# manikya7022/Continual-Learning-for-Dynamic-Video-Quality-Enhancement

Hardware: AMD Instinct MI355X
Metric: train frames/sec (2x SR, T=3, 540p->1080p) (higher is better)
Workload: dtype bf16

## Files before the change

continual-learning-for-dynamic-video-quality-enhancement_amd/csrc/aggregate.hip:

```cpp
#include "common.h"

namespace nvq {

__device__ __forceinline__ float sigmoidf_(float x) { return 1.f / (1.f + __expf(-x)); }

__device__ __forceinline__ float4 plane_reduce4b(float4 v, float4* buf, int C4, int npl) {
    __syncthreads();
    buf[threadIdx.x] = v;
    __syncthreads();
    float4 s = make_float4(0.f, 0.f, 0.f, 0.f);
    if ((int)threadIdx.x < C4)
        for (int k = 0; k < npl; ++k) {
            const float4 t = buf[k * C4 + threadIdx.x];
            s.x += t.x; s.y += t.y; s.z += t.z; s.w += t.w;
        }
    return s;
}

static inline int tsum_blocks_host(int H, int W) {
    int nb = ceil_div((long)H * W, 1024);
    if (nb > 256) nb = 256;
    if (nb < 1) nb = 1;
    return nb;
}
// ... 30 lines not shown
            const long pu = p0 + u * stride;
            if (pu >= HW) break;
            const long pix = base + pu;
            float mx = -3.4e38f;
#pragma unroll
            for (int t = 0; t < TMAX; ++t) mx = fmaxf(mx, lg[u][t]);
            float den = 0.f;
#pragma unroll
            for (int t = 0; t < TMAX; ++t) {
                lg[u][t] = t < T ? __expf(lg[u][t] - mx) : 0.f;
                den += lg[u][t];
            }
            const float inv = 1.f / den;
            float4 o = make_float4(0.f, 0.f, 0.f, 0.f);
#pragma unroll
            for (int t = 0; t < TMAX; ++t) {
                if (t < T) {
                    const float a = lg[u][t] * inv;
                    o.x += v[u][t].x * a; o.y += v[u][t].y * a; o.z += v[u][t].z * a; o.w += v[u][t].w * a;
                    if (c4 == 0) attn[pix * attn_ld + t] = a;
                }
            }
            if (c4 == 0)
                for (int t = T; t < attn_ld; ++t) attn[pix * attn_ld + t] = 0.f;
            stx4(weighted, pix * weighted_ld + 4 * c4, WB, o);
            gsum.x += o.x; gsum.y += o.y; gsum.z += o.z; gsum.w += o.w;
        }
    }
    const float4 r = plane_reduce4b(gsum, buf, C4, npl);
    if ((int)threadIdx.x < C4)
        st4(gap_partial + ((size_t)blockIdx.y * gridDim.x + blockIdx.x) * C + 4 * c4, r);
}

template <bool ALLB, bool WB>
__global__ __launch_bounds__(256) void tsum_bwd_kernel(const float* __restrict__ dweighted, int dweighted_ld,
                                                       const float* __restrict__ dgap_pix,
                                                       const float* __restrict__ aligned, int aligned_ld,
                                                       const float* __restrict__ attn, int attn_ld, int T, int C,
                                                       long HW, float* __restrict__ daligned, int daligned_ld,
                                                       float* __restrict__ dlogits, int dlogits_ld, long total,
                                                       int aligned_bf16_, int daligned_bf16_) {
    const int aligned_bf16 = ALLB ? 1 : aligned_bf16_, daligned_bf16 = ALLB ? 1 : daligned_bf16_;
    const long gid = blockIdx.x * 256L + threadIdx.x;
    if (gid >= total) return;
    const int C4 = C >> 2;
    const long pix = idiv(gid, C4, total);
    const int c4 = (int)(gid - pix * C4);
    const int n = (int)idiv(pix, HW, total);
    float4 dw = ldx4(dweighted, pix * dweighted_ld + 4 * c4, WB);
    if (dgap_pix) {
        const float4 gp = ld4(dgap_pix + (size_t)n * C + 4 * c4);
        dw.x += gp.x; dw.y += gp.y; dw.z += gp.z; dw.w += gp.w;
    }
    float a[NVQ_MAX_T], dot[NVQ_MAX_T];
    float sdot = 0.f;
#pragma unroll
    for (int t = 0; t < NVQ_MAX_T; ++t) {
        a[t] = 0.f; dot[t] = 0.f;
        if (t < T) {
            a[t] = attn[pix * attn_ld + t];
            const float4 v = ldx4(aligned, (size_t)pix * aligned_ld + t * C + 4 * c4, aligned_bf16);
            stx4(daligned, (size_t)pix * daligned_ld + t * C + 4 * c4, daligned_bf16,
                 make_float4(dw.x * a[t], dw.y * a[t], dw.z * a[t], dw.w * a[t]));
            dot[t] = group_sum(dw.x * v.x + dw.y * v.y + dw.z * v.z + dw.w * v.w, C4);
            sdot += a[t] * dot[t];
        }
    }
    if (c4 == 0) {
#pragma unroll
        for (int t = 0; t < NVQ_MAX_T; ++t)
            if (t < T) dlogits[pix * dlogits_ld + t] = a[t] * (dot[t] - sdot);
        for (int t = T; t < dlogits_ld; ++t) dlogits[pix * dlogits_ld + t] = 0.f;
    }
}

__global__ __launch_bounds__(256) void cbam_channel_kernel(const float* __restrict__ gap_partial, int nblk, int C,
                                                           int R, long HW, const float* __restrict__ w1,
                                                           const float* __restrict__ w2, float* __restrict__ gap,
                                                           float* __restrict__ hid, float* __restrict__ ca) {
    __shared__ float sg[256];
    __shared__ float sh[64];
    const int n = blockIdx.x, c = threadIdx.x;
    if (c < C) {
        double s = 0.0;
        const float* p = gap_partial + (size_t)n * nblk * C + c;
        for (int b = 0; b < nblk; ++b) s += (double)p[(size_t)b * C];
        const float g = (float)(s / (double)HW);
        sg[c] = g;
        gap[(size_t)n * C + c] = g;
    }
    __syncthreads();
    if (c < R) {
        float s = 0.f;
        for (int k = 0; k < C; ++k) s += w1[c * C + k] * sg[k];
        s = fmaxf(s, 0.f);
        sh[c] = s;
        hid[(size_t)n * R + c] = s;
    }
    __syncthreads();
    if (c < C) {
        float s = 0.f;
        for (int r = 0; r < R; ++r) s += w2[c * R + r] * sh[r];
        ca[(size_t)n * C + c] = sigmoidf_(s);
    }
}

template <bool XB>
__global__ __launch_bounds__(256) void cbam_pool_kernel(const float* __restrict__ x, int x_ld,
                                                        const float* __restrict__ ca, int C, long HW,
                                                        float* __restrict__ sm, int* __restrict__ amax, long total) {
    const long gid = blockIdx.x * 256L + threadIdx.x;
    if (gid >= total) return;
    const int C4 = C >> 2;
    const long pix = idiv(gid, C4, total);
    const int c4 = (int)(gid - pix * C4);
    const int n = (int)idiv(pix, HW, total);
    const float4 v = ldx4(x, pix * x_ld + 4 * c4, XB);
    const float4 a = ld4(ca + (size_t)n * C + 4 * c4);
    const float e[4] = {v.x * a.x, v.y * a.y, v.z * a.z, v.w * a.w};
    const float s = group_sum(e[0] + e[1] + e[2] + e[3], C4);
    float best = e[0];
    int bi = 4 * c4;
#pragma unroll
    for (int k = 1; k < 4; ++k)
        if (e[k] > best) { best = e[k]; bi = 4 * c4 + k; }
    for (int o = C4 >> 1; o > 0; o >>= 1) {
        const float ob = __shfl_xor(best, o, 64);
        const int oi = __shfl_xor(bi, o, 64);
        if (ob > best || (ob == best && oi < bi)) { best = ob; bi = oi; }
    }
    if (c4 == 0) {
        sm[pix * 2] = s / (float)C;
        sm[pix * 2 + 1] = best;
        amax[pix] = bi;
    }
}

constexpr int SP_T = 16;
constexpr int SP_H = SP_T + 6;

__global__ __launch_bounds__(256) void cbam_sa_kernel(const float* __restrict__ sm, const float* __restrict__ w7,
                                                      int H, int W, int tilesX, float* __restrict__ sa) {
    __shared__ float tile[2][SP_H][SP_H + 1];
    __shared__ float wl[98];
    const int n = blockIdx.y;
    const int ty0 = (blockIdx.x / tilesX) * SP_T, tx0 = (blockIdx.x % tilesX) * SP_T;
    if (threadIdx.x < 98) wl[threadIdx.x] = w7[threadIdx.x];
    for (int i = threadIdx.x; i < SP_H * SP_H; i += 256) {
        const int hy = i / SP_H, hx = i % SP_H;
        const int gy = ty0 + hy - 3, gx = tx0 + hx - 3;
        float a = 0.f, b = 0.f;
        if (gy >= 0 && gy < H && gx >= 0 && gx < W) {
            const size_t pix = (size_t)(n * H + gy) * W + gx;
            a = sm[pix * 2];
            b = sm[pix * 2 + 1];
        }
        tile[0][hy][hx] = a;
        tile[1][hy][hx] = b;
    }
    __syncthreads();
    const int py = threadIdx.x / SP_T, px = threadIdx.x % SP_T;
    const int gy = ty0 + py, gx = tx0 + px;
    if (gy >= H || gx >= W) return;
    float s = 0.f;
#pragma unroll
    for (int ch = 0; ch < 2; ++ch)
#pragma unroll
        for (int ky = 0; ky < 7; ++ky)
#pragma unroll
            for (int kx = 0; kx < 7; ++kx) s += wl[(ch * 7 + ky) * 7 + kx] * tile[ch][py + ky][px + kx];
    sa[(size_t)(n * H + gy) * W + gx] = sigmoidf_(s);
}

template <bool XB>
__global__ __launch_bounds__(256) void cbam_apply_kernel(const float* __restrict__ x, int x_ld,
                                                         const float* __restrict__ ca, const float* __restrict__ sa,
                                                         int C, long HW, float* __restrict__ out, int out_ld,
                                                         int out_coff, int out_bf16, long total) {
    const long gid = blockIdx.x * 256L + threadIdx.x;
    if (gid >= total) return;
    const int C4 = C >> 2;
    const long pix = idiv(gid, C4, total);
    const int c4 = (int)(gid - pix * C4);
    const int n = (int)idiv(pix, HW, total);
    const float4 v = ldx4(x, pix * x_ld + 4 * c4, XB);
    const float4 a = ld4(ca + (size_t)n * C + 4 * c4);
    const float s = sa[pix];
    const float4 o = make_float4(v.x * a.x * s, v.y * a.y * s, v.z * a.z * s, v.w * a.w * s);
    if (out_bf16) {
        typedef __bf16 bf16x4_t __attribute__((ext_vector_type(4)));
        *reinterpret_cast<bf16x4_t*>(reinterpret_cast<__bf16*>(out) + pix * out_ld + out_coff + 4 * c4) =
            (bf16x4_t){(__bf16)o.x, (__bf16)o.y, (__bf16)o.z, (__bf16)o.w};
    } else {
        st4(out + pix * out_ld + out_coff + 4 * c4, o);
    }
}

template <bool XB>
__global__ __launch_bounds__(256) void cbam_bwd_pre_kernel(const float* __restrict__ dout, int dout_ld, int dout_coff,
                                                           const float* __restrict__ x, int x_ld,
                                                           const float* __restrict__ ca, const float* __restrict__ sa,
                                                           int C, long HW, float* __restrict__ dpre, long total) {
    const long gid = blockIdx.x * 256L + threadIdx.x;
    if (gid >= total) return;
    const int C4 = C >> 2;
    const long pix = idiv(gid, C4, total);
    const int c4 = (int)(gid - pix * C4);
    const int n = (int)idiv(pix, HW, total);
    const float4 g = ldx4(dout, pix * dout_ld + dout_coff + 4 * c4, XB);
    const float4 v = ldx4(x, pix * x_ld + 4 * c4, XB);
    const float4 a = ld4(ca + (size_t)n * C + 4 * c4);
    const float d = group_sum(g.x * v.x * a.x + g.y * v.y * a.y + g.z * v.z * a.z + g.w * v.w * a.w, C4);
    if (c4 == 0) {
        const float s = sa[pix];
        dpre[pix] = d * s * (1.f - s);
    }
}

template <bool WG>
__global__ __launch_bounds__(256) void cbam_bwd_conv_kernel(const float* __restrict__ dpre,
                                                            const float* __restrict__ sm,
                                                            const float* __restrict__ w7, int H, int W, int tilesX,
                                                            float* __restrict__ dsm, float* __restrict__ part) {
    __shared__ float dtile[SP_H][SP_H + 1];
    __shared__ float stile[2][SP_H][SP_H + 1];
    __shared__ float wl[98];
    const int n = blockIdx.y;
    const int ty0 = (blockIdx.x / tilesX) * SP_T, tx0 = (blockIdx.x % tilesX) * SP_T;
    if (threadIdx.x < 98) wl[threadIdx.x] = w7[threadIdx.x];
    for (int i = threadIdx.x; i < SP_H * SP_H; i += 256) {
        const int hy = i / SP_H, hx = i % SP_H;
        const int gy = ty0 + hy - 3, gx = tx0 + hx - 3;
        float d = 0.f, a = 0.f, b = 0.f;
        if (gy >= 0 && gy < H && gx >= 0 && gx < W) {
            const size_t pix = (size_t)(n * H + gy) * W + gx;
            d = dpre[pix];
            if constexpr (WG) {
                a = sm[pix * 2];
                b = sm[pix * 2 + 1];
            }
        }
        dtile[hy][hx] = d;
        if constexpr (WG) {
            stile[0][hy][hx] = a;
            stile[1][hy][hx] = b;
        }
    }
    __syncthreads();
    const int py = threadIdx.x / SP_T, px = threadIdx.x % SP_T;
    const int gy = ty0 + py, gx = tx0 + px;
    if (gy < H && gx < W) {
        float s0 = 0.f, s1 = 0.f;
#pragma unroll
        for (int ky = 0; ky < 7; ++ky)
#pragma unroll
            for (int kx = 0; kx < 7; ++kx) {
                const float d = dtile[py + 6 - ky][px + 6 - kx];
                s0 += wl[ky * 7 + kx] * d;
                s1 += wl[49 + ky * 7 + kx] * d;
            }
        const size_t pix = (size_t)(n * H + gy) * W + gx;
        dsm[pix * 2] = s0;
        dsm[pix * 2 + 1] = s1;
    }
    if (WG && threadIdx.x < 98) {
        const int ch = threadIdx.x / 49, ky = (threadIdx.x % 49) / 7, kx = threadIdx.x % 7;
        float s = 0.f;
        for (int yy = 0; yy < SP_T; ++yy)
            for (int xx = 0; xx < SP_T; ++xx) s += stile[ch][yy + ky][xx + kx] * dtile[yy + 3][xx + 3];
        part[((size_t)blockIdx.y * gridDim.x + blockIdx.x) * 98 + threadIdx.x] = s;
    }
}

template <bool XB>
__global__ __launch_bounds__(256) void cbam_bwd_scale_kernel(const float* __restrict__ dout, int dout_ld, int dout_coff,
                                                             const float* __restrict__ x, int x_ld,
                                                             const float* __restrict__ ca, const float* __restrict__ sa,
                                                             const float* __restrict__ dsm, const int* __restrict__ amax,
                                                             int C, long HW, float* __restrict__ dx, int dx_ld,
                                                             float* __restrict__ dca_partial) {
    __shared__ float4 buf[256];
    const int C4 = C >> 2;
    const int npl = 256 / C4;
    const int c4 = threadIdx.x % C4, pl = threadIdx.x / C4;
    const int n = blockIdx.y;
    const long base = (long)n * HW;
    const float4 a = ld4(ca + (size_t)n * C + 4 * c4);
    const float invC = 1.f / (float)C;
    float4 acc = make_float4(0.f, 0.f, 0.f, 0.f);
    for (long p = (long)blockIdx.x * npl + pl; p < HW; p += (long)gridDim.x * npl) {
        const long pix = base + p;
        const float4 g = ldx4(dout, pix * dout_ld + dout_coff + 4 * c4, XB);
        const float4 v = ldx4(x, pix * x_ld + 4 * c4, XB);
        const float s = sa[pix];
        const float d0 = dsm[pix * 2] * invC, d1 = dsm[pix * 2 + 1];
        const int am = amax[pix] - 4 * c4;
        float4 dxc;
        dxc.x = g.x * s + d0 + (am == 0 ? d1 : 0.f);
        dxc.y = g.y * s + d0 + (am == 1 ? d1 : 0.f);
        dxc.z = g.z * s + d0 + (am == 2 ? d1 : 0.f);
        dxc.w = g.w * s + d0 + (am == 3 ? d1 : 0.f);
        stx4(dx, pix * dx_ld + 4 * c4, XB, make_float4(dxc.x * a.x, dxc.y * a.y, dxc.z * a.z, dxc.w * a.w));
        acc.x += dxc.x * v.x; acc.y += dxc.y * v.y; acc.z += dxc.z * v.z; acc.w += dxc.w * v.w;
    }
    const float4 r = plane_reduce4b(acc, buf, C4, npl);
    if ((int)threadIdx.x < C4)
        st4(dca_partial + ((size_t)n * gridDim.x + blockIdx.x) * C + 4 * c4, r);
}

template <bool WG>
__global__ __launch_bounds__(256) void cbam_bwd_channel_kernel(const float* __restrict__ dca_partial, int nblk, int C,
                                                               int R, int N, long HW, const float* __restrict__ w1,
                                                               const float* __restrict__ w2, const float* __restrict__ gap,
                                                               const float* __restrict__ hid, const float* __restrict__ ca,
                                                               float* __restrict__ dw1, float* __restrict__ dw2,
                                                               float* __restrict__ dgap_pix, int accumulate) {
    __shared__ float dz2[256];
    __shared__ float dz1[16];
    __shared__ float sh[16];
    const int c = threadIdx.x;
    float a1[16], a2[16];
#pragma unroll
    for (int r = 0; r < 16; ++r) { a1[r] = 0.f; a2[r] = 0.f; }
    __shared__ double sp[256];
    const int parts = 256 / C;
    for (int n = 0; n < N; ++n) {
        __syncthreads();
        {
            const int cc = c % C, part = c / C;
            double s = 0.0;
            if (part < parts) {
                const float* p = dca_partial + (size_t)n * nblk * C + cc;
                for (int b = part; b < nblk; b += parts) s += (double)p[(size_t)b * C];
            }
            sp[c] = s;
        }
        __syncthreads();
        float z = 0.f;
        if (c < C) {
            double s = 0.0;
            for (int k = 0; k < parts; ++k) s += sp[k * C + c];
            const float cav = ca[(size_t)n * C + c];
            z = (float)s * cav * (1.f - cav);
        }
        dz2[c] = z;
        if (c < R) sh[c] = hid[(size_t)n * R + c];
        __syncthreads();
        if (c < R) {
            float s = 0.f;
            for (int k = 0; k < C; ++k) s += w2[k * R + c] * dz2[k];
            dz1[c] = sh[c] > 0.f ? s : 0.f;
        }
        __syncthreads();
        if (c < C) {
            const float gv = gap[(size_t)n * C + c];
            float dg = 0.f;
#pragma unroll
            for (int r = 0; r < 16; ++r)
                if (r < R) {
                    if constexpr (WG) {
                        a2[r] += z * sh[r];
                        a1[r] += dz1[r] * gv;
                    }
                    dg += w1[r * C + c] * dz1[r];
                }
            dgap_pix[(size_t)n * C + c] = dg / (float)HW;
        }
    }
    if (WG && c < C) {
#pragma unroll
        for (int r = 0; r < 16; ++r)
            if (r < R) {
                dw2[c * R + r] = accumulate ? dw2[c * R + r] + a2[r] : a2[r];
                dw1[r * C + c] = accumulate ? dw1[r * C + c] + a1[r] : a1[r];
            }
    }
}

static bool pow2_c4(int C) {
    const int c4 = C >> 2;
    return C % 4 == 0 && c4 >= 1 && c4 <= 64 && (c4 & (c4 - 1)) == 0;
}

}

using namespace nvq;

extern "C" {

int nvq_tsum_blocks(int H, int W) { return tsum_blocks_host(H, W); }

int nvq_tsum_forward(const float* aligned, int aligned_ld, const float* logits, int logits_ld, int T, int C,
                     int N, int H, int W, float* attn, int attn_ld, float* weighted, int weighted_ld,
                     float* gap_partial, int aligned_bf16, int weighted_bf16, void* stream) {
    NVQ_REQUIRE(pow2_c4(C), "tsum_forward: C %d must be a power of two in [4,256]", C);
    NVQ_REQUIRE(T >= 1 && T <= NVQ_MAX_T && logits_ld >= T && attn_ld >= T, "tsum_forward: T %d", T);
    NVQ_REQUIRE(aligned_ld % 4 == 0 && weighted_ld % 4 == 0 && aligned_ld >= T * C, "tsum_forward: ld");
    const dim3 grid(tsum_blocks_host(H, W), N);
    with_bools([&](auto SMALL, auto AB, auto WB) {
        constexpr int M = SMALL() ? 4 : NVQ_MAX_T, U = SMALL() ? 4 : 2;
        hipLaunchKernelGGL((tsum_fwd_kernel<M, U, AB(), WB()>), grid, dim3(256), 0, (hipStream_t)stream, aligned, aligned_ld, logits,
                           logits_ld, T, C, (long)H * W, attn, attn_ld, weighted, weighted_ld, gap_partial);
    }, T <= 4, aligned_bf16, weighted_bf16);
    return check_launch("tsum_forward");
}

int nvq_tsum_backward(const float* dweighted, int dweighted_ld, const float* dgap_pix, const float* aligned,
                      int aligned_ld, const float* attn, int attn_ld, int T, int C, int N, int H, int W,
                      float* daligned, int daligned_ld, float* dlogits, int dlogits_ld, int aligned_bf16,
                      int daligned_bf16, int dweighted_bf16, void* stream) {
    NVQ_REQUIRE(pow2_c4(C), "tsum_backward: C %d must be a power of two in [4,256]", C);
    NVQ_REQUIRE(T >= 1 && T <= NVQ_MAX_T && dlogits_ld >= T && attn_ld >= T, "tsum_backward: T %d", T);
    NVQ_REQUIRE(aligned_ld % 4 == 0 && dweighted_ld % 4 == 0 && daligned_ld % 4 == 0, "tsum_backward: ld");
    const long total = (long)N * H * W * (C / 4);
    with_bools([&](auto AB, auto WB) {
        hipLaunchKernelGGL((tsum_bwd_kernel<AB(), WB()>), dim3(ceil_div(total, 256)), dim3(256), 0, (hipStream_t)stream, dweighted,
                           dweighted_ld, dgap_pix, aligned, aligned_ld, attn, attn_ld, T, C, (long)H * W, daligned, daligned_ld, dlogits,
                           dlogits_ld, total, aligned_bf16, daligned_bf16);
    }, aligned_bf16 && daligned_bf16, dweighted_bf16);
    return check_launch("tsum_backward");
}

int nvq_cbam_channel(const float* gap_partial, int nblk, int C, int R, int N, int HW, const float* w1,
                     const float* w2, float* gap, float* hid, float* ca, void* stream) {
    NVQ_REQUIRE(C <= 256 && R >= 1 && R <= 16, "cbam_channel: C %d R %d", C, R);
    hipLaunchKernelGGL(cbam_channel_kernel, dim3(N), dim3(256), 0, (hipStream_t)stream, gap_partial, nblk, C, R,
                       (long)HW, w1, w2, gap, hid, ca);
    return check_launch("cbam_channel");
}

int nvq_cbam_pool(const float* x, int x_ld, const float* ca, int C, int N, int H, int W, float* sm, int* amax,
                  int x_bf16, void* stream) {
    NVQ_REQUIRE(pow2_c4(C) && x_ld % 4 == 0, "cbam_pool: C %d must be a power of two in [4,256]", C);
    const long total = (long)N * H * W * (C / 4);
    if (x_bf16)
        hipLaunchKernelGGL(cbam_pool_kernel<true>, dim3(ceil_div(total, 256)), dim3(256), 0, (hipStream_t)stream, x, x_ld, ca, C,
                           (long)H * W, sm, amax, total);
    else
        hipLaunchKernelGGL(cbam_pool_kernel<false>, dim3(ceil_div(total, 256)), dim3(256), 0, (hipStream_t)stream, x, x_ld, ca, C,
                           (long)H * W, sm, amax, total);
    return check_launch("cbam_pool");
}

int nvq_cbam_spatial_apply(const float* x, int x_ld, const float* ca, const float* sm, const float* w7, int C,
                           int N, int H, int W, float* sa, float* out, int out_ld, int out_coff, int out_bf16,
                           int x_bf16, void* stream) {
    NVQ_REQUIRE(C % 4 == 0 && x_ld % 4 == 0 && out_ld % 4 == 0 && out_coff % 4 == 0, "cbam_spatial_apply: alignment");
    const int tilesX = (W + SP_T - 1) / SP_T, tilesY = (H + SP_T - 1) / SP_T;
    hipStream_t s = (hipStream_t)stream;
    hipLaunchKernelGGL(cbam_sa_kernel, dim3(tilesX * tilesY, N), dim3(256), 0, s, sm, w7, H, W, tilesX, sa);
    int rc = check_launch("cbam_sa");
    if (rc) return rc;
    const long total = (long)N * H * W * (C / 4);
    if (x_bf16)
        hipLaunchKernelGGL(cbam_apply_kernel<true>, dim3(ceil_div(total, 256)), dim3(256), 0, s, x, x_ld, ca, sa, C, (long)H * W,
                           out, out_ld, out_coff, out_bf16, total);
    else
        hipLaunchKernelGGL(cbam_apply_kernel<false>, dim3(ceil_div(total, 256)), dim3(256), 0, s, x, x_ld, ca, sa, C, (long)H * W,
                           out, out_ld, out_coff, out_bf16, total);
    return check_launch("cbam_apply");
}

int nvq_cbam_bwd_spatial_pre(const float* dout, int dout_ld, int dout_coff, const float* x, int x_ld,
                             const float* ca, const float* sa, int C, int N, int H, int W, float* dpre,
                             int x_bf16, void* stream) {
    NVQ_REQUIRE(pow2_c4(C) && x_ld % 4 == 0 && dout_ld % 4 == 0 && dout_coff % 4 == 0,
                "cbam_bwd_spatial_pre: C %d must be a power of two in [4,256]", C);
    const long total = (long)N * H * W * (C / 4);
    if (x_bf16)
        hipLaunchKernelGGL(cbam_bwd_pre_kernel<true>, dim3(ceil_div(total, 256)), dim3(256), 0, (hipStream_t)stream, dout, dout_ld,
                           dout_coff, x, x_ld, ca, sa, C, (long)H * W, dpre, total);
    else
        hipLaunchKernelGGL(cbam_bwd_pre_kernel<false>, dim3(ceil_div(total, 256)), dim3(256), 0, (hipStream_t)stream, dout, dout_ld,
                           dout_coff, x, x_ld, ca, sa, C, (long)H * W, dpre, total);
    return check_launch("cbam_bwd_spatial_pre");
}

int nvq_cbam_bwd_spatial_conv_ex(const float* dpre, const float* sm, const float* w7, int N, int H, int W, float* dsm,
                                 float* dw7, float* workspace, size_t workspace_bytes, int accumulate, int flags, void* stream) {
    NVQ_REQUIRE((flags & ~NVQ_NO_WGRAD) == 0, "cbam_bwd_spatial_conv_ex: flags %d", flags);
    const bool wg = !(flags & NVQ_NO_WGRAD);
    const int tilesX = (W + SP_T - 1) / SP_T, tilesY = (H + SP_T - 1) / SP_T;
    const int nblk = tilesX * tilesY * N;
    hipStream_t s = (hipStream_t)stream;
    if (!wg) {
        hipLaunchKernelGGL(cbam_bwd_conv_kernel<false>, dim3(tilesX * tilesY, N), dim3(256), 0, s, dpre, sm, w7, H, W, tilesX,
                           dsm, workspace);
        return check_launch("cbam_bwd_spatial_conv");
    }
    if ((size_t)nblk * 98 * sizeof(float) > workspace_bytes) { set_error("cbam_bwd_spatial_conv: workspace"); return NVQ_EWORKSPACE; }
    hipLaunchKernelGGL(cbam_bwd_conv_kernel<true>, dim3(tilesX * tilesY, N), dim3(256), 0, s, dpre, sm, w7, H, W, tilesX, dsm,
                       workspace);
    int rc = check_launch("cbam_bwd_spatial_conv");
    if (rc) return rc;
    return launch_reduce_partials(workspace, nblk, 98, 1.f, dw7, accumulate, s);
}

int nvq_cbam_bwd_spatial_conv(const float* dpre, const float* sm, const float* w7, int N, int H, int W, float* dsm,
                              float* dw7, float* workspace, size_t workspace_bytes, int accumulate, void* stream) {
    return nvq_cbam_bwd_spatial_conv_ex(dpre, sm, w7, N, H, W, dsm, dw7, workspace, workspace_bytes, accumulate, 0, stream);
}

int nvq_cbam_bwd_scale(const float* dout, int dout_ld, int dout_coff, const float* x, int x_ld, const float* ca,
                       const float* sa, const float* dsm, const int* amax, int C, int N, int H, int W, float* dx,
                       int dx_ld, float* dca_partial, int x_bf16, void* stream) {
    NVQ_REQUIRE(pow2_c4(C) && x_ld % 4 == 0 && dout_ld % 4 == 0 && dout_coff % 4 == 0 && dx_ld % 4 == 0,
                "cbam_bwd_scale: C %d must be a power of two in [4,256]", C);
    if (x_bf16)
        hipLaunchKernelGGL(cbam_bwd_scale_kernel<true>, dim3(tsum_blocks_host(H, W), N), dim3(256), 0, (hipStream_t)stream, dout,
                           dout_ld, dout_coff, x, x_ld, ca, sa, dsm, amax, C, (long)H * W, dx, dx_ld, dca_partial);
    else
        hipLaunchKernelGGL(cbam_bwd_scale_kernel<false>, dim3(tsum_blocks_host(H, W), N), dim3(256), 0, (hipStream_t)stream, dout,
                           dout_ld, dout_coff, x, x_ld, ca, sa, dsm, amax, C, (long)H * W, dx, dx_ld, dca_partial);
    return check_launch("cbam_bwd_scale");
}

int nvq_cbam_bwd_channel_ex(const float* dca_partial, int nblk, int C, int R, int N, int HW, const float* w1,
                            const float* w2, const float* gap, const float* hid, const float* ca, float* dw1,
                            float* dw2, float* dgap_pix, int accumulate, int flags, void* stream) {
    NVQ_REQUIRE((flags & ~NVQ_NO_WGRAD) == 0, "cbam_bwd_channel_ex: flags %d", flags);
    NVQ_REQUIRE(C <= 256 && R >= 1 && R <= 16, "cbam_bwd_channel: C %d R %d", C, R);
    if (flags & NVQ_NO_WGRAD)
        hipLaunchKernelGGL(cbam_bwd_channel_kernel<false>, dim3(1), dim3(256), 0, (hipStream_t)stream, dca_partial, nblk, C, R, N,
                           (long)HW, w1, w2, gap, hid, ca, dw1, dw2, dgap_pix, accumulate);
    else
        hipLaunchKernelGGL(cbam_bwd_channel_kernel<true>, dim3(1), dim3(256), 0, (hipStream_t)stream, dca_partial, nblk, C, R, N,
                           (long)HW, w1, w2, gap, hid, ca, dw1, dw2, dgap_pix, accumulate);
    return check_launch("cbam_bwd_channel");
}

int nvq_cbam_bwd_channel(const float* dca_partial, int nblk, int C, int R, int N, int HW, const float* w1,
                         const float* w2, const float* gap, const float* hid, const float* ca, float* dw1,
                         float* dw2, float* dgap_pix, int accumulate, void* stream) {
    return nvq_cbam_bwd_channel_ex(dca_partial, nblk, C, R, N, HW, w1, w2, gap, hid, ca, dw1, dw2, dgap_pix, accumulate, 0, stream);
}

}
```

continual-learning-for-dynamic-video-quality-enhancement_amd/csrc/common.h:

```cpp
#pragma once
#include <hip/hip_runtime.h>
#include <stdarg.h>
#include <stdio.h>
#include <type_traits>
#include "../../include/nvq.h"

namespace nvq {

void set_error(const char* fmt, ...);

inline int check_launch(const char* what) {
    hipError_t e = hipGetLastError();
    if (e != hipSuccess) {
        set_error("%s: %s", what, hipGetErrorString(e));
        return NVQ_ELAUNCH;
    }
    return NVQ_OK;
}

#define NVQ_REQUIRE(cond, ...)            \
    do {                                  \
        if (!(cond)) {                    \
            nvq::set_error(__VA_ARGS__);  \
            return NVQ_EINVAL;            \
// ... 2 lines not shown

inline bool aligned16(const void* p) { return (reinterpret_cast<uintptr_t>(p) & 15) == 0; }
inline bool aligned8(const void* p) { return (reinterpret_cast<uintptr_t>(p) & 7) == 0; }
inline bool aligned4(const void* p) { return (reinterpret_cast<uintptr_t>(p) & 3) == 0; }
inline int ceil_div(long a, long b) { return (int)((a + b - 1) / b); }

template <bool... Bs, class F>
inline void with_bools(F&& f) {
    f(std::bool_constant<Bs>{}...);
}
template <bool... Bs, class F, class... Rest>
inline void with_bools(F&& f, bool b, Rest... rest) {
    if (b) with_bools<Bs..., true>(f, rest...);
    else with_bools<Bs..., false>(f, rest...);
}

template <int... Vs>
struct one_of {
    int v;
    explicit one_of(int v_) : v(v_) {}
};
template <class... Ks, class F, class... Rest>
inline int with_consts(const char*, F&&, bool, Rest...);
template <class... Ks, class F, class... Rest>
inline int with_consts(const char*, F&&, one_of<>, Rest...);
template <class... Ks, class F, int V, int... Vs, class... Rest>
inline int with_consts(const char*, F&&, one_of<V, Vs...>, Rest...);

template <class... Ks, class F>
inline int with_consts(const char*, F&& f) {
    f(Ks{}...);
    return NVQ_OK;
}
template <class... Ks, class F, class... Rest>
inline int with_consts(const char* what, F&& f, bool b, Rest... rest) {
    return b ? with_consts<Ks..., std::true_type>(what, f, rest...) : with_consts<Ks..., std::false_type>(what, f, rest...);
}
template <class... Ks, class F, class... Rest>
inline int with_consts(const char* what, F&&, one_of<> a, Rest...) {
    set_error("%s: no kernel form for the value %d", what, a.v);
    return NVQ_EINVAL;
}
template <class... Ks, class F, int V, int... Vs, class... Rest>
inline int with_consts(const char* what, F&& f, one_of<V, Vs...> a, Rest... rest) {
    return a.v == V ? with_consts<Ks..., std::integral_constant<int, V>>(what, f, rest...)
                    : with_consts<Ks...>(what, f, one_of<Vs...>(a.v), rest...);
}

typedef float f32x4 __attribute__((ext_vector_type(4)));

__device__ __forceinline__ float4 ld4(const float* p) { return *reinterpret_cast<const float4*>(p); }
__device__ __forceinline__ void st4(float* p, float4 v) { *reinterpret_cast<float4*>(p) = v; }

typedef __bf16 bf16x8 __attribute__((ext_vector_type(8)));
typedef __bf16 bf16x4 __attribute__((ext_vector_type(4)));

__device__ __forceinline__ float4 ldx4(const float* base, size_t idx, int is_bf16) {
    if (is_bf16) {
        const bf16x4 v = *reinterpret_cast<const bf16x4*>(reinterpret_cast<const __bf16*>(base) + idx);
        return make_float4((float)v[0], (float)v[1], (float)v[2], (float)v[3]);
    }
    return ld4(base + idx);
}
__device__ __forceinline__ void stx4(float* base, size_t idx, int is_bf16, float4 v) {
    if (is_bf16)
        *reinterpret_cast<bf16x4*>(reinterpret_cast<__bf16*>(base) + idx) =
            (bf16x4){(__bf16)v.x, (__bf16)v.y, (__bf16)v.z, (__bf16)v.w};
    else
        st4(base + idx, v);
}

__device__ __forceinline__ long idiv(long a, int d, long total) {
    return total <= 0xffffffffL ? (long)((unsigned)a / (unsigned)d) : a / d;
}
__device__ __forceinline__ long idiv(long a, long d, long total) {
    return (total <= 0xffffffffL && d <= 0xffffffffL) ? (long)((unsigned)a / (unsigned)d) : a / d;
}

__device__ __forceinline__ float group_sum(float v, int width) {
    for (int o = width >> 1; o > 0; o >>= 1) v += __shfl_xor(v, o, 64);
    return v;
}

__device__ __forceinline__ float block_sum_256(float v, float* scratch) {
    v = group_sum(v, 64);
    const int wave = threadIdx.x >> 6;
    __syncthreads();
    if ((threadIdx.x & 63) == 0) scratch[wave] = v;
    __syncthreads();
    return scratch[0] + scratch[1] + scratch[2] + scratch[3];
}

__device__ __forceinline__ int xcd_tile(int bid, int n) {
    const int q = n >> 3, r = n & 7, x = bid & 7;
    return x * q + (x < r ? x : r) + (bid >> 3);
}

int launch_reduce_partials(const float* part, int nblk, int K, float alpha, float* out,
                           int accumulate, hipStream_t s);

}
```

continual-learning-for-dynamic-video-quality-enhancement_amd/csrc/conv_igemm.hip:

```cpp
#include "conv_common.h"
#include "flat.h"

namespace nvq {

constexpr int KC = 16;
constexpr int XS_LD = 20;

__device__ __forceinline__ float pack_f32_elem(const float* __restrict__ w, int cout_w, int cin_w, int taps, int transpose,
                                               int cout_keep, int NT, int nkc, long idx) {
    long t = idx;
    const int j = t & 3; t >>= 2;
    const int n = t % NT; t /= NT;
    const int g = t & 3; t >>= 2;
    const int tap = t % taps; t /= taps;
    const int kc = t % nkc; t /= nkc;
    const int cz = (int)t;
    const int co = cz * NT + n;
    const int ch = kc * KC + 4 * g + j;
    float v = 0.f;
    if (!transpose) {
        if (co < cout_w && ch < cin_w) v = w[((long)co * cin_w + ch) * taps + tap];
    } else {
        if (co < cout_keep && ch < cout_w) v = w[((long)ch * cin_w + co) * taps + (taps - 1 - tap)];
    }
// ... 339 lines not shown
            }
            for (; k < nsplit; k += WR_Q) s4[0] += (double)part[(size_t)k * total + idx];
        }
        sh[q][e] = (s4[0] + s4[1]) + (s4[2] + s4[3]);
        __syncthreads();
        if (q == 0 && idx < total) {
            double sum = 0.0;
#pragma unroll
            for (int u = 0; u < WR_Q; ++u) sum += sh[u][e];
            long t = idx;
            const int col = t % WG_C; t /= WG_C;
            const int cil = t % WG_C; t /= WG_C;
            const int tap = t % taps; t /= taps;
            const int coc = t % nco;
            const int cic = (int)(t / nco);
            const int ci = cic * WG_C + cil, co = coc * WG_C + col;
            if (ci < cin_w && co < cout) {
                const float v = alpha * (float)sum;
                const long o = ((long)co * cin_w + ci) * taps + tap;
                dw[o] = accumulate ? dw[o] + v : v;
            }
        }
        __syncthreads();
    }
}

__global__ __launch_bounds__(256) void wgrad_reduce_kernel(const float* __restrict__ part, int nsplit, int nci, int nco,
                                                           int taps, int cout, int cin_w, float alpha, int accumulate,
                                                           float* __restrict__ dw, int wblocks, const float* __restrict__ bp,
                                                           float* __restrict__ dbias) {
    __shared__ double sh[WR_Q][WR_E];
    wgrad_reduce_body(part, nsplit, nci, nco, taps, cout, cin_w, alpha, accumulate, dw, wblocks, bp, dbias, (int)blockIdx.x, sh);
}

constexpr int WR_MAX_JOBS = 16;
struct WgradReduceTable { nvq_wgrad_reduce_job j[WR_MAX_JOBS]; };
__global__ __launch_bounds__(256) void wgrad_reduce_batch_kernel(const WgradReduceTable t) {
    __shared__ double sh[WR_Q][WR_E];
    const nvq_wgrad_reduce_job& j = t.j[blockIdx.y];
    const long total = (long)j.nci * j.nco * j.taps * WG_C * WG_C;
    const int bblk = j.dbias ? (j.cout + 3) / 4 : 0;
    long nblk = (total + WR_E - 1) / WR_E;
    if (nblk > (long)gridDim.x - bblk) nblk = (long)gridDim.x - bblk;
    if ((int)blockIdx.x >= nblk + bblk) return;
    wgrad_reduce_body(j.part, j.nsplit, j.nci, j.nco, j.taps, j.cout, j.cin_w, j.alpha, j.accumulate, j.dw, (int)nblk,
                      j.bias_part, j.dbias, (int)blockIdx.x, sh);
}

static int launch_wgrad_reduce_bias(const float* part, int nsplit, int nci, int nco, int taps, int cout, int cin_w, float alpha,
                                    int accumulate, float* dw, const float* bias_part, float* dbias, hipStream_t s) {
    const long total = (long)nci * nco * taps * WG_C * WG_C;
    int nblk = ceil_div(total, WR_E);
    if (nblk > 4096) nblk = 4096;
    const int bblk = dbias ? ceil_div(cout, 4) : 0;
    hipLaunchKernelGGL(wgrad_reduce_kernel, dim3(nblk + bblk), dim3(256), 0, s, part, nsplit, nci, nco, taps, cout, cin_w, alpha,
                       accumulate, dw, nblk, bias_part, dbias);
    return check_launch("conv_wgrad_reduce");
}
int launch_wgrad_reduce(const float* part, int nsplit, int nci, int nco, int taps, int cout, int cin_w, float alpha,
                        int accumulate, float* dw, hipStream_t s) {
    return launch_wgrad_reduce_bias(part, nsplit, nci, nco, taps, cout, cin_w, alpha, accumulate, dw, nullptr, nullptr, s);
}

__global__ __launch_bounds__(256) void colsum_kernel(const float* __restrict__ x, int ld, int coff,
                                                     int C, int CP, long npix,
                                                     float* __restrict__ part) {
    __shared__ float red[256];
    const int c = threadIdx.x % CP;
    const int pl = threadIdx.x / CP;
    const int lanes = 256 / CP;
    float s = 0.f;
    if (c < C)
        for (long p = (long)blockIdx.x * lanes + pl; p < npix; p += (long)gridDim.x * lanes)
            s += x[p * ld + coff + c];
    red[threadIdx.x] = s;
    __syncthreads();
    if (pl == 0 && c < C) {
        float t = 0.f;
        for (int k = 0; k < lanes; ++k) t += red[k * CP + c];
        part[(long)blockIdx.x * C + c] = t;
    }
}

__global__ __launch_bounds__(256) void reduce_partials_kernel(const float* __restrict__ part, int nblk, int K,
                                                              float alpha, float* __restrict__ out, int accumulate) {
    const int k = blockIdx.x * 4 + (threadIdx.x >> 6);
    const int lane = threadIdx.x & 63;
    if (k >= K) return;
    double s = 0.0;
    for (int b = lane; b < nblk; b += 64) s += (double)part[(long)b * K + k];
    s = wave_sum(s);
    if (lane == 0) {
        const float v = alpha * (float)s;
        out[k] = accumulate ? out[k] + v : v;
    }
}

int launch_reduce_partials(const float* part, int nblk, int K, float alpha, float* out,
                           int accumulate, hipStream_t s) {
    hipLaunchKernelGGL(reduce_partials_kernel, dim3(ceil_div(K, 4)), dim3(256), 0, s, part, nblk,
                       K, alpha, out, accumulate);
    return check_launch("reduce_partials");
}

static int colsum_impl(const float* x, int ld, int coff, int C, long npix, float alpha, float* out,
                       float* ws, size_t ws_bytes, int accumulate, hipStream_t s) {
    NVQ_REQUIRE(C >= 1 && C <= 256, "colsum: C=%d out of range", C);
    int CP = 1;
    while (CP < C) CP <<= 1;
    const int lanes = 256 / CP;
    int nblk = ceil_div(npix, (long)lanes * 8);
    if (nblk > 512) nblk = 512;
    if (nblk < 1) nblk = 1;
    if ((size_t)nblk * C * sizeof(float) > ws_bytes) {
        set_error("colsum: workspace too small");
        return NVQ_EWORKSPACE;
    }
    hipLaunchKernelGGL(colsum_kernel, dim3(nblk), dim3(256), 0, s, x, ld, coff, C, CP, npix, ws);
    int rc = check_launch("colsum");
    if (rc) return rc;
    return launch_reduce_partials(ws, nblk, C, alpha, out, accumulate, s);
}

}

using namespace nvq;

extern "C" {

size_t nvq_conv_pack_floats(int cout, int cin_store, int ksize, int math) {
    if (math == NVQ_MATH_BF16) return pack_floats_bf16(cout, cin_store, ksize);
    const int NT = choose_nt(cout);
    const size_t ncz = (cout + NT - 1) / NT, nkc = (cin_store + KC - 1) / KC;
    return ncz * nkc * (size_t)(ksize * ksize) * 4 * NT * 4;
}

int nvq_conv_pack(const float* w, int cout_w, int cin_w, int ksize, int transpose, int cin_store,
                  int cout_keep, int math, float* wpack, void* stream) {
    NVQ_REQUIRE(ksize == 1 || ksize == 3, "conv_pack: ksize %d", ksize);
    const int cout = transpose ? cout_keep : cout_w;
    const int cin_real = transpose ? cout_w : cin_w;
    NVQ_REQUIRE(cin_store >= cin_real && cin_store % 4 == 0, "conv_pack: cin_store %d < %d or not %%4",
                cin_store, cin_real);
    NVQ_REQUIRE(!transpose || cout_keep <= cin_w, "conv_pack: cout_keep %d > cin_w %d", cout_keep, cin_w);
    NVQ_REQUIRE(math == NVQ_MATH_F32 || math == NVQ_MATH_BF16, "conv_pack: math mode %d", math);
    if (math == NVQ_MATH_BF16)
        return pack_bf16(w, cout_w, cin_w, ksize, transpose, cin_store, cout_keep, wpack, (hipStream_t)stream);
    const int NT = choose_nt(cout);
    const int ncz = (cout + NT - 1) / NT, nkc = (cin_store + KC - 1) / KC;
    const long total = (long)ncz * nkc * ksize * ksize * 4 * NT * 4;
    int nblk = ceil_div(total, 256);
    if (nblk > 2048) nblk = 2048;
    hipLaunchKernelGGL(pack_kernel, dim3(nblk), dim3(256), 0, (hipStream_t)stream, w, cout_w, cin_w,
                       ksize * ksize, transpose, cout_keep, NT, ncz, nkc, wpack);
    return check_launch("conv_pack");
}

int nvq_conv_pack_batch(const nvq_pack_job* jobs, int njobs, int math, void* stream) {
    NVQ_REQUIRE(njobs >= 0 && (njobs == 0 || jobs), "conv_pack_batch: %d jobs", njobs);
    NVQ_REQUIRE(math == NVQ_MATH_F32 || math == NVQ_MATH_BF16, "conv_pack_batch: math mode %d", math);
    for (int i = 0; i < njobs; ++i) {
        const nvq_pack_job& j = jobs[i];
        NVQ_REQUIRE(j.ksize == 1 || j.ksize == 3, "conv_pack_batch[%d]: ksize %d", i, j.ksize);
        const int cin_real = j.transpose ? j.cout_w : j.cin_w;
        NVQ_REQUIRE(j.cin_store >= cin_real && j.cin_store % 4 == 0, "conv_pack_batch[%d]: cin_store %d < %d or not %%4", i,
                    j.cin_store, cin_real);
        NVQ_REQUIRE(!j.transpose || j.cout_keep <= j.cin_w, "conv_pack_batch[%d]: cout_keep %d > cin_w %d", i, j.cout_keep,
                    j.cin_w);
        NVQ_REQUIRE(j.w && j.wpack, "conv_pack_batch[%d]: null pointer", i);
    }
    hipStream_t s = (hipStream_t)stream;
    for (int base = 0; base < njobs; base += PACK_BATCH) {
        const int n = njobs - base < PACK_BATCH ? njobs - base : PACK_BATCH;
        PackJobTable t{};
        for (int i = 0; i < n; ++i) {
            const nvq_pack_job& j = jobs[base + i];
            if (math == NVQ_MATH_BF16) {
                t.j[i] = pack_job_bf16(j);
            } else {
                const int cout = j.transpose ? j.cout_keep : j.cout_w;
                const int NT = choose_nt(cout);
                const int ncz = (cout + NT - 1) / NT, nkc = (j.cin_store + KC - 1) / KC;
                t.j[i] = PackJobDev{j.w, j.wpack, j.cout_w, j.cin_w, j.ksize * j.ksize, j.transpose, j.cout_keep, NT, ncz, nkc,
                                    (long)ncz * nkc * j.ksize * j.ksize * 4 * NT * 4};
// ... 267 lines not shown
```

continual-learning-for-dynamic-video-quality-enhancement_amd/csrc/reduce.hip:

```cpp
#include "flat.h"

namespace nvq {

__global__ __launch_bounds__(256) void group_final_kernel(const float* __restrict__ part, int nblk, double alpha, double bias,
                                                          float* __restrict__ out) {
    __shared__ double scratch[256];
    const float* p = part + (long)blockIdx.x * nblk;
    double s = 0.0;
    for (int k = threadIdx.x; k < nblk; k += 256) s += (double)p[k];
    s = block_tree_sum_256(s, scratch);
    if (threadIdx.x == 0) out[blockIdx.x] = (float)(bias + alpha * s);
}

void launch_group_final(const float* part, int nblk, int groups, double alpha, double bias, float* out, hipStream_t s) {
    hipLaunchKernelGGL(group_final_kernel, dim3(groups), dim3(256), 0, s, part, nblk, alpha, bias, out);
}

__global__ void serial_final_kernel(const float* __restrict__ part, int nblk, double alpha, float* __restrict__ out) {
    if (threadIdx.x == 0 && blockIdx.x == 0) {
        double s = 0.0;
        for (int k = 0; k < nblk; ++k) s += (double)part[k];
        *out = (float)(alpha * s);
    }
}

void launch_serial_final(const float* part, int nblk, double alpha, float* out, hipStream_t s) {
    hipLaunchKernelGGL(serial_final_kernel, dim3(1), dim3(64), 0, s, part, nblk, alpha, out);
}

}
```

Measured before the change: 80.27.

## Batch CBAM per-pixel kernels, use DPP reductions, and unroll ordered partial sums

The CBAM pool and backward-pre kernels now handle four pixel groups per thread, and their cross-lane sums and argmax use DPP moves instead of generic shuffles. Partial-sum reductions in the channel kernels, reduce_partials and serial_final load many values ahead in unrolled batches while keeping the sequential double-precision summation order. The channel backward kernel caches w1/w2 in registers and LDS and processes several images per iteration. These target latency-bound small reductions and kernel overhead, at the cost of more code, more registers and more shared memory.

Result: no change. 80.73, median of 6 (+0.6%).

```diff
diff --git a/continual-learning-for-dynamic-video-quality-enhancement_amd/csrc/aggregate.hip b/continual-learning-for-dynamic-video-quality-enhancement_amd/csrc/aggregate.hip
--- a/continual-learning-for-dynamic-video-quality-enhancement_amd/csrc/aggregate.hip
+++ b/continual-learning-for-dynamic-video-quality-enhancement_amd/csrc/aggregate.hip
@@ -136,9 +136,7 @@
     __shared__ float sh[64];
     const int n = blockIdx.x, c = threadIdx.x;
     if (c < C) {
-        double s = 0.0;
-        const float* p = gap_partial + (size_t)n * nblk * C + c;
-        for (int b = 0; b < nblk; ++b) s += (double)p[(size_t)b * C];
+        const double s = ordered_sum<16>(0.0, gap_partial + (size_t)n * nblk * C + c, C, nblk);
         const float g = (float)(s / (double)HW);
         sg[c] = g;
         gap[(size_t)n * C + c] = g;
@@ -159,34 +157,105 @@
     }
 }
 
+template <int O>
+__device__ __forceinline__ int lane_xor_i(int v) {
+    if constexpr (O == 1) return __builtin_amdgcn_mov_dpp(v, 0xB1, 0xF, 0xF, true);
+    else if constexpr (O == 2) return __builtin_amdgcn_mov_dpp(v, 0x4E, 0xF, 0xF, true);
+    else if constexpr (O == 4) {
+        const int t = __builtin_amdgcn_update_dpp(v, v, 0x104, 0xF, 0x5, false);
+        return __builtin_amdgcn_update_dpp(t, v, 0x114, 0xF, 0xA, false);
+    } else if constexpr (O == 8) return __builtin_amdgcn_mov_dpp(v, 0x128, 0xF, 0xF, true);
+    else return __shfl_xor(v, O, 64);
+}
+template <int O>
+__device__ __forceinline__ float lane_xor_f(float v) { return __int_as_float(lane_xor_i<O>(__float_as_int(v))); }
+
+template <class F>
+__device__ __forceinline__ void xor_steps(int width, F&& f) {
+    if (width > 32) f.template operator()<32>();
+    if (width > 16) f.template operator()<16>();
+    if (width > 8) f.template operator()<8>();
+    if (width > 4) f.template operator()<4>();
+    if (width > 2) f.template operator()<2>();
+    if (width > 1) f.template operator()<1>();
+}
+
+struct GroupSumStep {
+    float& v;
+    template <int O> __device__ __forceinline__ void operator()() { v += lane_xor_f<O>(v); }
+};
+__device__ __forceinline__ float group_sum_dpp(float v, int width) {
+    xor_steps(width, GroupSumStep{v});
+    return v;
+}
+
+struct ArgmaxStep {
+    float& best;
+    int& bi;
+    template <int O> __device__ __forceinline__ void operator()() {
+        const float ob = lane_xor_f<O>(best);
+        const int oi = lane_xor_i<O>(bi);
+        if (ob > best || (ob == best && oi < bi)) { best = ob; bi = oi; }
+    }
+};
+
+constexpr int CBAM_PU = 4;
+struct CbamItems {
+    long pix[CBAM_PU];
+    int n[CBAM_PU];
+    bool live[CBAM_PU];
+    int c4;
+};
+__device__ __forceinline__ CbamItems cbam_items(long gid0, int C4, long HW, long total) {
+    CbamItems it;
+    const int sh = __builtin_ctz(C4), npl = 256 >> sh;
+    const long pix0 = gid0 >> sh;
+    const int n0 = (int)idiv(pix0, HW, total);
+    const long r0 = pix0 - n0 * HW;
+    it.c4 = (int)(gid0 & (C4 - 1));
+#pragma unroll
+    for (int u = 0; u < CBAM_PU; ++u) {
+        it.live[u] = gid0 + u * 256 < total;
+        long r = r0 + u * npl;
+        int n = n0;
+        while (r >= HW) { r -= HW; ++n; }
+        it.pix[u] = it.live[u] ? pix0 + u * npl : pix0;
+        it.n[u] = it.live[u] ? n : n0;
+    }
+    return it;
+}
+
 template <bool XB>
 __global__ __launch_bounds__(256) void cbam_pool_kernel(const float* __restrict__ x, int x_ld,
                                                         const float* __restrict__ ca, int C, long HW,
                                                         float* __restrict__ sm, int* __restrict__ amax, long total) {
-    const long gid = blockIdx.x * 256L + threadIdx.x;
-    if (gid >= total) return;
+    const long gid0 = (long)blockIdx.x * (256 * CBAM_PU) + threadIdx.x;
+    if (gid0 >= total) return;
     const int C4 = C >> 2;
-    const long pix = idiv(gid, C4, total);
-    const int c4 = (int)(gid - pix * C4);
-    const int n = (int)idiv(pix, HW, total);
-    const float4 v = ldx4(x, pix * x_ld + 4 * c4, XB);
-    const float4 a = ld4(ca + (size_t)n * C + 4 * c4);
-    const float e[4] = {v.x * a.x, v.y * a.y, v.z * a.z, v.w * a.w};
-    const float s = group_sum(e[0] + e[1] + e[2] + e[3], C4);
-    float best = e[0];
-    int bi = 4 * c4;
-#pragma unroll
-    for (int k = 1; k < 4; ++k)
-        if (e[k] > best) { best = e[k]; bi = 4 * c4 + k; }
-    for (int o = C4 >> 1; o > 0; o >>= 1) {
-        const float ob = __shfl_xor(best, o, 64);
-        const int oi = __shfl_xor(bi, o, 64);
-        if (ob > best || (ob == best && oi < bi)) { best = ob; bi = oi; }
-    }
-    if (c4 == 0) {
-        sm[pix * 2] = s / (float)C;
-        sm[pix * 2 + 1] = best;
-        amax[pix] = bi;
+    const CbamItems it = cbam_items(gid0, C4, HW, total);
+    const int c4 = it.c4;
+    float4 v[CBAM_PU], a[CBAM_PU];
+#pragma unroll
+    for (int u = 0; u < CBAM_PU; ++u) {
+        v[u] = ldx4(x, it.pix[u] * x_ld + 4 * c4, XB);
+        a[u] = ld4(ca + (size_t)it.n[u] * C + 4 * c4);
+    }
+#pragma unroll
+    for (int u = 0; u < CBAM_PU; ++u) {
+        const float e[4] = {v[u].x * a[u].x, v[u].y * a[u].y, v[u].z * a[u].z, v[u].w * a[u].w};
+        const float s = group_sum_dpp(e[0] + e[1] + e[2] + e[3], C4);
+        float best = e[0];
+        int bi = 4 * c4;
+#pragma unroll
+        for (int k = 1; k < 4; ++k)
+            if (e[k] > best) { best = e[k]; bi = 4 * c4 + k; }
+        xor_steps(C4, ArgmaxStep{best, bi});
+        if (c4 == 0 && it.live[u]) {
+            const long pix = it.pix[u];
+            sm[pix * 2] = s / (float)C;
+            sm[pix * 2 + 1] = best;
+            amax[pix] = bi;
+        }
     }
 }
 
@@ -255,19 +324,28 @@
                                                            const float* __restrict__ x, int x_ld,
                                                            const float* __restrict__ ca, const float* __restrict__ sa,
                                                            int C, long HW, float* __restrict__ dpre, long total) {
-    const long gid = blockIdx.x * 256L + threadIdx.x;
-    if (gid >= total) return;
+    const long gid0 = (long)blockIdx.x * (256 * CBAM_PU) + threadIdx.x;
+    if (gid0 >= total) return;
     const int C4 = C >> 2;
-    const long pix = idiv(gid, C4, total);
-    const int c4 = (int)(gid - pix * C4);
-    const int n = (int)idiv(pix, HW, total);
-    const float4 g = ldx4(dout, pix * dout_ld + dout_coff + 4 * c4, XB);
-    const float4 v = ldx4(x, pix * x_ld + 4 * c4, XB);
-    const float4 a = ld4(ca + (size_t)n * C + 4 * c4);
-    const float d = group_sum(g.x * v.x * a.x + g.y * v.y * a.y + g.z * v.z * a.z + g.w * v.w * a.w, C4);
-    if (c4 == 0) {
-        const float s = sa[pix];
-        dpre[pix] = d * s * (1.f - s);
+    const CbamItems it = cbam_items(gid0, C4, HW, total);
+    const int c4 = it.c4;
+    float4 g[CBAM_PU], v[CBAM_PU], a[CBAM_PU];
+    float sv[CBAM_PU];
+#pragma unroll
+    for (int u = 0; u < CBAM_PU; ++u) {
+        g[u] = ldx4(dout, it.pix[u] * dout_ld + dout_coff + 4 * c4, XB);
+        v[u] = ldx4(x, it.pix[u] * x_ld + 4 * c4, XB);
+        a[u] = ld4(ca + (size_t)it.n[u] * C + 4 * c4);
+        sv[u] = c4 == 0 ? sa[it.pix[u]] : 0.f;
+    }
+#pragma unroll
+    for (int u = 0; u < CBAM_PU; ++u) {
+        const float d = group_sum_dpp(g[u].x * v[u].x * a[u].x + g[u].y * v[u].y * a[u].y + g[u].z * v[u].z * a[u].z +
+                                      g[u].w * v[u].w * a[u].w, C4);
+        if (c4 == 0 && it.live[u]) {
+            const float s = sv[u];
+            dpre[it.pix[u]] = d * s * (1.f - s);
+        }
     }
 }
 
@@ -362,6 +440,7 @@
         st4(dca_partial + ((size_t)n * gridDim.x + blockIdx.x) * C + 4 * c4, r);
 }
 
+constexpr int CBC_NB = 8;
 template <bool WG>
 __global__ __launch_bounds__(256) void cbam_bwd_channel_kernel(const float* __restrict__ dca_partial, int nblk, int C,
                                                                int R, int N, long HW, const float* __restrict__ w1,
@@ -371,54 +450,64 @@
                                                                float* __restrict__ dgap_pix, int accumulate) {
     __shared__ float dz2[256];
     __shared__ float dz1[16];
-    __shared__ float sh[16];
+    __shared__ float sh[CBC_NB][16];
+    __shared__ float w2l[256 * 16];
     const int c = threadIdx.x;
-    float a1[16], a2[16];
-#pragma unroll
-    for (int r = 0; r < 16; ++r) { a1[r] = 0.f; a2[r] = 0.f; }
-    __shared__ double sp[256];
+    float a1[16], a2[16], w1r[16];
+#pragma unroll
+    for (int r = 0; r < 16; ++r) { a1[r] = 0.f; a2[r] = 0.f; w1r[r] = (r < R && c < C) ? w1[r * C + c] : 0.f; }
+    for (int i = c; i < C * R; i += 256) w2l[i] = w2[i];
+    __shared__ double sp[CBC_NB][256];
     const int parts = 256 / C;
-    for (int n = 0; n < N; ++n) {
+    for (int n0 = 0; n0 < N; n0 += CBC_NB) {
+        const int nb = N - n0 < CBC_NB ? N - n0 : CBC_NB;
+        float cav[CBC_NB], gv[CBC_NB];
         __syncthreads();
-        {
+#pragma unroll
+        for (int i = 0; i < CBC_NB; ++i) {
+            cav[i] = (i < nb && c < C) ? ca[(size_t)(n0 + i) * C + c] : 0.f;
+            gv[i] = (i < nb && c < C) ? gap[(size_t)(n0 + i) * C + c] : 0.f;
+            if (i < nb && c < R) sh[i][c] = hid[(size_t)(n0 + i) * R + c];
+        }
+        for (int i = 0; i < nb; ++i) {
             const int cc = c % C, part = c / C;
             double s = 0.0;
-            if (part < parts) {
-                const float* p = dca_partial + (size_t)n * nblk * C + cc;
-                for (int b = part; b < nblk; b += parts) s += (double)p[(size_t)b * C];
-            }
-            sp[c] = s;
-        }
-        __syncthreads();
-        float z = 0.f;
-        if (c < C) {
-            double s = 0.0;
-            for (int k = 0; k < parts; ++k) s += sp[k * C + c];
-            const float cav = ca[(size_t)n * C + c];
-            z = (float)s * cav * (1.f - cav);
-        }
-        dz2[c] = z;
-        if (c < R) sh[c] = hid[(size_t)n * R + c];
-        __syncthreads();
-        if (c < R) {
-            float s = 0.f;
-            for (int k = 0; k < C; ++k) s += w2[k * R + c] * dz2[k];
-            dz1[c] = sh[c] > 0.f ? s : 0.f;
-        }
-        __syncthreads();
-        if (c < C) {
-            const float gv = gap[(size_t)n * C + c];
-            float dg = 0.f;
-#pragma unroll
-            for (int r = 0; r < 16; ++r)
-                if (r < R) {
-                    if constexpr (WG) {
-                        a2[r] += z * sh[r];
-                        a1[r] += dz1[r] * gv;
+            if (part < parts && part < nblk)
+                s = ordered_sum<16>(0.0, dca_partial + ((size_t)(n0 + i) * nblk + part) * C + cc, (long)parts * C,
+                                    (nblk - part + parts - 1) / parts);
+            sp[i][c] = s;
+        }
+#pragma unroll
+        for (int i = 0; i < CBC_NB; ++i) {
+            if (i >= nb) break;
+            __syncthreads();
+            float z = 0.f;
+            if (c < C) {
+                double s = 0.0;
+                for (int k = 0; k < parts; ++k) s += sp[i][k * C + c];
+                z = (float)s * cav[i] * (1.f - cav[i]);
+            }
+            dz2[c] = z;
+            __syncthreads();
+            if (c < R) {
+                float s = 0.f;
+                for (int k = 0; k < C; ++k) s += w2l[k * R + c] * dz2[k];
+                dz1[c] = sh[i][c] > 0.f ? s : 0.f;
+            }
+            __syncthreads();
+            if (c < C) {
+                float dg = 0.f;
+#pragma unroll
+                for (int r = 0; r < 16; ++r)
+                    if (r < R) {
+                        if constexpr (WG) {
+                            a2[r] += z * sh[i][r];
+                            a1[r] += dz1[r] * gv[i];
+                        }
+                        dg += w1r[r] * dz1[r];
                     }
-                    dg += w1[r * C + c] * dz1[r];
-                }
-            dgap_pix[(size_t)n * C + c] = dg / (float)HW;
+                dgap_pix[(size_t)(n0 + i) * C + c] = dg / (float)HW;
+            }
         }
     }
     if (WG && c < C) {
@@ -488,10 +577,10 @@
     NVQ_REQUIRE(pow2_c4(C) && x_ld % 4 == 0, "cbam_pool: C %d must be a power of two in [4,256]", C);
     const long total = (long)N * H * W * (C / 4);
     if (x_bf16)
-        hipLaunchKernelGGL(cbam_pool_kernel<true>, dim3(ceil_div(total, 256)), dim3(256), 0, (hipStream_t)stream, x, x_ld, ca, C,
+        hipLaunchKernelGGL(cbam_pool_kernel<true>, dim3(ceil_div(total, 256L * CBAM_PU)), dim3(256), 0, (hipStream_t)stream, x, x_ld, ca, C,
                            (long)H * W, sm, amax, total);
     else
-        hipLaunchKernelGGL(cbam_pool_kernel<false>, dim3(ceil_div(total, 256)), dim3(256), 0, (hipStream_t)stream, x, x_ld, ca, C,
+        hipLaunchKernelGGL(cbam_pool_kernel<false>, dim3(ceil_div(total, 256L * CBAM_PU)), dim3(256), 0, (hipStream_t)stream, x, x_ld, ca, C,
                            (long)H * W, sm, amax, total);
     return check_launch("cbam_pool");
 }
@@ -522,10 +611,10 @@
                 "cbam_bwd_spatial_pre: C %d must be a power of two in [4,256]", C);
     const long total = (long)N * H * W * (C / 4);
     if (x_bf16)
-        hipLaunchKernelGGL(cbam_bwd_pre_kernel<true>, dim3(ceil_div(total, 256)), dim3(256), 0, (hipStream_t)stream, dout, dout_ld,
+        hipLaunchKernelGGL(cbam_bwd_pre_kernel<true>, dim3(ceil_div(total, 256L * CBAM_PU)), dim3(256), 0, (hipStream_t)stream, dout, dout_ld,
                            dout_coff, x, x_ld, ca, sa, C, (long)H * W, dpre, total);
     else
-        hipLaunchKernelGGL(cbam_bwd_pre_kernel<false>, dim3(ceil_div(total, 256)), dim3(256), 0, (hipStream_t)stream, dout, dout_ld,
+        hipLaunchKernelGGL(cbam_bwd_pre_kernel<false>, dim3(ceil_div(total, 256L * CBAM_PU)), dim3(256), 0, (hipStream_t)stream, dout, dout_ld,
                            dout_coff, x, x_ld, ca, sa, C, (long)H * W, dpre, total);
     return check_launch("cbam_bwd_spatial_pre");
 }
diff --git a/continual-learning-for-dynamic-video-quality-enhancement_amd/csrc/common.h b/continual-learning-for-dynamic-video-quality-enhancement_amd/csrc/common.h
--- a/continual-learning-for-dynamic-video-quality-enhancement_amd/csrc/common.h
+++ b/continual-learning-for-dynamic-video-quality-enhancement_amd/csrc/common.h
@@ -108,6 +108,34 @@
     return v;
 }
 
+template <int U>
+__device__ __forceinline__ double ordered_sum_trips(double s, const float* __restrict__ p, long stride, int n, int& done) {
+    int i = done;
+    for (; i + U <= n; i += U) {
+        float v[U];
+#pragma unroll
+        for (int u = 0; u < U; ++u) v[u] = p[(long)(i + u) * stride];
+#pragma unroll
+        for (int u = 0; u < U; ++u) s += (double)v[u];
+    }
+    done = i;
+    return s;
+}
+template <int U>
+__device__ __forceinline__ double ordered_sum(double s, const float* __restrict__ p, long stride, int n) {
+    int i = 0;
+    s = ordered_sum_trips<U>(s, p, stride, n, i);
+    if (i < n) {
+        float v[U];
+#pragma unroll
+        for (int u = 0; u < U; ++u) v[u] = p[(long)(i + u < n ? i + u : n - 1) * stride];
+#pragma unroll
+        for (int u = 0; u < U; ++u)
+            if (i + u < n) s += (double)v[u];
+    }
+    return s;
+}
+
 __device__ __forceinline__ float block_sum_256(float v, float* scratch) {
     v = group_sum(v, 64);
     const int wave = threadIdx.x >> 6;
diff --git a/continual-learning-for-dynamic-video-quality-enhancement_amd/csrc/conv_igemm.hip b/continual-learning-for-dynamic-video-quality-enhancement_amd/csrc/conv_igemm.hip
--- a/continual-learning-for-dynamic-video-quality-enhancement_amd/csrc/conv_igemm.hip
+++ b/continual-learning-for-dynamic-video-quality-enhancement_amd/csrc/conv_igemm.hip
@@ -445,12 +445,17 @@
     }
 }
 
-__global__ __launch_bounds__(256) void reduce_partials_kernel(const float* __restrict__ part, int nblk, int K,
-                                                              float alpha, float* __restrict__ out, int accumulate) {
-    const int k = blockIdx.x * 4 + (threadIdx.x >> 6);
-    const int lane = threadIdx.x & 63;
-    if (k >= K) return;
+__global__ __launch_bounds__(64) void reduce_partials_kernel(const float* __restrict__ part, int nblk, int K,
+                                                             float alpha, float* __restrict__ out, int accumulate) {
+    const int k = blockIdx.x;
+    const int lane = threadIdx.x;
+    const int rows = nblk > lane ? (nblk - lane + 63) >> 6 : 0;
+    int done = 0;
     double s = 0.0;
+    s = ordered_sum_trips<16>(s, part + (long)lane * K + k, 64L * K, rows, done);
+    s = ordered_sum_trips<4>(s, part + (long)lane * K + k, 64L * K, rows, done);
+    part += (long)done * 64 * K;
+    nblk -= done * 64;
     for (int b = lane; b < nblk; b += 64) s += (double)part[(long)b * K + k];
     s = wave_sum(s);
     if (lane == 0) {
@@ -461,8 +466,7 @@
 
 int launch_reduce_partials(const float* part, int nblk, int K, float alpha, float* out,
                            int accumulate, hipStream_t s) {
-    hipLaunchKernelGGL(reduce_partials_kernel, dim3(ceil_div(K, 4)), dim3(256), 0, s, part, nblk,
-                       K, alpha, out, accumulate);
+    hipLaunchKernelGGL(reduce_partials_kernel, dim3(K), dim3(64), 0, s, part, nblk, K, alpha, out, accumulate);
     return check_launch("reduce_partials");
 }
 
diff --git a/continual-learning-for-dynamic-video-quality-enhancement_amd/csrc/reduce.hip b/continual-learning-for-dynamic-video-quality-enhancement_amd/csrc/reduce.hip
--- a/continual-learning-for-dynamic-video-quality-enhancement_amd/csrc/reduce.hip
+++ b/continual-learning-for-dynamic-video-quality-enhancement_amd/csrc/reduce.hip
@@ -16,12 +16,30 @@
     hipLaunchKernelGGL(group_final_kernel, dim3(groups), dim3(256), 0, s, part, nblk, alpha, bias, out);
 }
 
-__global__ void serial_final_kernel(const float* __restrict__ part, int nblk, double alpha, float* __restrict__ out) {
-    if (threadIdx.x == 0 && blockIdx.x == 0) {
-        double s = 0.0;
-        for (int k = 0; k < nblk; ++k) s += (double)part[k];
-        *out = (float)(alpha * s);
+constexpr int SF_U = 8;
+__global__ __launch_bounds__(64) void serial_final_kernel(const float* __restrict__ part, int nblk, double alpha,
+                                                          float* __restrict__ out) {
+    const int lane = threadIdx.x;
+    double s = 0.0;
+    for (int k0 = 0; k0 < nblk; k0 += SF_U * 64) {
+        float v[SF_U];
+#pragma unroll
+        for (int u = 0; u < SF_U; ++u) {
+            const int k = k0 + u * 64 + lane;
+            v[u] = part[k < nblk ? k : nblk - 1];
+        }
+#pragma unroll
+        for (int u = 0; u < SF_U; ++u) {
+            const int left = nblk - (k0 + u * 64);
+            if (left >= 64) {
+#pragma unroll
+                for (int j = 0; j < 64; ++j) s += (double)__int_as_float(__builtin_amdgcn_readlane(__float_as_int(v[u]), j));
+            } else {
+                for (int j = 0; j < left; ++j) s += (double)__int_as_float(__builtin_amdgcn_readlane(__float_as_int(v[u]), j));
+            }
+        }
     }
+    if (lane == 0) *out = (float)(alpha * s);
 }
 
 void launch_serial_final(const float* part, int nblk, double alpha, float* out, hipStream_t s) {
```
